# chunhualiao/Smith-Waterman

Hardware: AMD Instinct MI355X
Metric: GCUPS (DP cell updates/s) on NxN random DNA pair (higher is better)
Workload: dtype int32; 1 GPU; 16384x16384 random DNA pair (reference generator, seed 1+rank), linear gap 3/-3/-2, int32 H + int32 P written to HBM, arg-max tracked; per_gpu=one pair per GPU, max_pos=268369846, max_score=11583, grid=256, column_tiles=1, strips=131, placement_held_gib=0, preheat_fills=620

## Files before the change

### smith-waterman_amd/csrc/sw_api.hip

```cpp
#include <hip/hip_runtime.h>
#include <algorithm>
#include <chrono>
#include <cstdio>
#include <cstdlib>
#include <cstring>
#include <iterator>
#include <map>
#include <mutex>
#include <string>
#include <thread>
#include <vector>
#include "sw_kernels.h"
#include "sw_plan.h"

namespace swh { void set_err(const char* fmt, ...); }
extern "C" int sw_place_pair_ratio(void* d_X, size_t xbytes, void* d_Y, size_t ybytes, float* ratio, float* ms_together);
using swh::set_err;

#define HIP_TRY(expr)                                                                 \
    do {                                                                              \
        hipError_t e_ = (expr);                                                       \
        if (e_ != hipSuccess) {                                                       \
            set_err("%s failed: %s (%s:%d)", #expr, hipGetErrorString(e_), __FILE__, __LINE__); \
            return SW_EDEVICE;                                                        \
// ... 7 lines not shown
    hipEvent_t ev = nullptr;
    int concurrent_ok = 0;
};
static DevState g_dev[64];

struct sw_ctx {
    int device = 0;
    int num_cus = 256;
    unsigned epoch = 0;
    unsigned long long* d_edge = nullptr;
    size_t edge_cap = 0;
    unsigned long long* d_key = nullptr;
    unsigned long long* d_keys = nullptr; size_t keys_cap = 0;
    unsigned char* d_cb = nullptr;
    size_t cb_cap = 0;
    unsigned int* d_edge4 = nullptr;
    size_t edge4_cap = 0;
    unsigned epoch8 = 0;
    unsigned char* d_alpha = nullptr;
    unsigned int* d_part = nullptr;
    unsigned int* d_sync = nullptr;
    unsigned char* d_priv = nullptr; size_t priv_cap = 0;
    int64_t opt_place_hold_gib = 0;
    int64_t opt_place_budget_ms = 1500;
    int place_spacer_gib = 0;
    int64_t last_place_held_gib = 0;
    float last_place_ratio = 0.f;
    bool key_dirty = false;
    bool last_fused = false;
    swp::PlanOptions opt;
    swp::FillPlan last_plan;
    int64_t last_grid = 0;
    int s2_per_cu = 0;
    int64_t opt_xcd_order = 0;
    int64_t opt_pace_ps = 0;
    int64_t opt_dbg_ptr = 0;
    int64_t opt_band_wait_ms = 20000;
    unsigned char* d_bcodes = nullptr; size_t bcodes_cap = 0;
    int* d_bnd = nullptr; size_t bnd_cap = 0;
    int64_t opt_batch_lds = 0;
    int64_t last_batch_kernel = 0;
    signed char* d_sprof = nullptr; size_t sprof_cap = 0;
    int* d_sbnd = nullptr; size_t sbnd_cap = 0;
    swk::SearchItem* d_sitems = nullptr; swk::SearchItem* h_sitems = nullptr; size_t sitems_cap = 0;
    hipEvent_t sitems_ev = nullptr;
    unsigned int* d_sctr = nullptr;
    int64_t last_search_grid = 0;
    int64_t last_search_kernel = 0;
    int search_per_cu[swp::kSearchKernels] = {};
    bool search_per_cu_known = false;
    bool xcd_round_robin = false;
    std::map<void*, void*> out_base;
    std::map<void*, float> pair_ratio;
};

template <typename K> struct Indexed { int index; K k; };
template <typename K, size_t N> constexpr bool at_their_indices(const Indexed<K> (&t)[N]) {
    for (size_t i = 0; i < N; ++i)
        if (t[i].index != (int)i) return false;
    return true;
}

extern "C" {

int sw_create(int device, sw_ctx** out) {
    if (!out) { set_err("sw_create: out is NULL"); return SW_EINVAL; }
// ... 82 lines not shown
    if (!strcmp(name, "engine")) {
        if (v != 0 && v != 1) { set_err("engine must be 0 (systolic) or 1 (strip_scan)"); return SW_EINVAL; }
        c->opt.engine = v;
        return SW_OK;
    }
    set_err("sw_set_option: unknown option '%s'", name);
    return SW_EINVAL;
}

int64_t sw_get_option(sw_ctx* c, const char* name) {
    if (!c || !name) return -1;
    if (!strcmp(name, "waves_per_block")) return c->opt.waves_per_block;
    if (!strcmp(name, "max_blocks")) return c->opt.max_blocks;
    if (!strcmp(name, "engine")) return c->opt.engine;
    if (!strcmp(name, "strips_per_group")) return c->opt.strips_per_group;
    if (!strcmp(name, "consumers")) return c->opt.consumers;
    if (!strcmp(name, "store_policy")) return c->opt.store_policy;
    if (!strcmp(name, "xcd_order")) return c->opt_xcd_order;
    if (!strcmp(name, "importers")) return c->opt.importers;
    if (!strcmp(name, "pace_ps")) return c->opt_pace_ps;
    if (!strcmp(name, "band_wait_ms")) return c->opt_band_wait_ms;
    if (!strcmp(name, "num_cus")) return c->num_cus;
    if (!strcmp(name, "debug_edge4_ptr")) return (int64_t)(uintptr_t)c->d_edge4;
    if (!strcmp(name, "debug_edge4_cap")) return (int64_t)c->edge4_cap;
    if (!strcmp(name, "last_grid")) return c->last_grid;
    const swp::TilePlan& last_tile = c->last_plan.tile[c->last_plan.ntile - 1];
    if (!strcmp(name, "last_strips")) return c->last_plan.S;
    if (!strcmp(name, "last_strips2")) return last_tile.strips;
    if (!strcmp(name, "last_perm")) return c->last_plan.perm ? 1 : 0;
    if (!strcmp(name, "last_scouts")) return last_tile.nscout;
    if (!strcmp(name, "last_xcd_mode")) return last_tile.xcd_mode;
    if (!strcmp(name, "last_tiles")) return c->last_plan.ntile;
    if (!strcmp(name, "last_split_from")) return last_tile.split_blk ? last_tile.split_from : 0;
    if (!strcmp(name, "xcd_round_robin")) return c->xcd_round_robin ? 1 : 0;
    if (!strcmp(name, "last_batch_kernel")) return c->last_batch_kernel;
    if (!strcmp(name, "last_search_grid")) return c->last_search_grid;
    if (!strcmp(name, "last_search_kernel")) return c->last_search_kernel;
    if (!strcmp(name, "placement_budget_ms")) return c->opt_place_budget_ms;
    if (!strcmp(name, "placement_hold_gib")) return c->opt_place_hold_gib;
    if (!strcmp(name, "probe_foreign_pairs")) return c->opt.probe_foreign_pairs;
    if (!strcmp(name, "last_placement_held_gib")) return c->last_place_held_gib;
    if (!strcmp(name, "last_placement_ratio_x1000")) return (int64_t)(c->last_place_ratio * 1000.f);
    return -1;
}

static int check_dims(int64_t cols, int64_t rows, const sw_scores* sc, int64_t gc = -1, int64_t gr = -1) {
    if (gc < cols) gc = cols;
    if (gr < rows) gr = rows;
    if (cols < 0 || rows < 0 || cols > swk::SW_MAX_DIM || rows > swk::SW_MAX_DIM || gc > swk::SW_MAX_DIM || gr > swk::SW_MAX_DIM) {
        set_err("dimensions out of range: cols=%lld rows=%lld (max %lld)", (long long)cols, (long long)rows,
                (long long)swk::SW_MAX_DIM);
        return SW_EINVAL;
    }
    if (sc->gap > 0) { set_err("gap score must be <= 0 (got %d)", sc->gap); return SW_EINVAL; }
    if (sc->match < 0) { set_err("match score must be >= 0 (got %d)", sc->match); return SW_EINVAL; }
    if (sc->mismatch > sc->match) { set_err("mismatch score must not exceed the match score"); return SW_EINVAL; }
    const int64_t lo = std::min(gc, gr);
    const int64_t gmax = (int64_t)sc->match * lo + (int64_t)(-sc->gap) * (rows + cols + 2);
    const int64_t step = std::max<int64_t>(std::llabs((int64_t)sc->mismatch), (int64_t)sc->match) + 2 * (int64_t)(-sc->gap);
    if (gmax + step >= (1ll << 31) || step >= (1ll << 24) || (int64_t)sc->match * lo >= (1ll << 24)) {
        set_err("scores too large for this problem size (32-bit cell / 24-bit arg-max key)");
        return SW_EINVAL;
    }
    return SW_OK;
}

// ... 168 lines not shown
    unsigned short* d_cb16 = (unsigned short*)(c->d_cb + cb16);
    unsigned char* d_cbc = c->d_cb + cb16 + ((2 * c->cb_cap + 15) / 16) * 16;
    if (plan.perm) {
        p.edge4 = c->d_edge4; p.e4stride = plan.e4stride; p.edge4_pstride = S * plan.e4stride;
        p.gbias = next_gbias(c, stream);
    }
    p.bcode = d_cbc;
    p.atab = c->d_alpha + 64;
    p.phi_base = plan.fast ? (int)S - 1 : -1;
    p.bfront = (int)plan.bfront;
    p.bpad16 = d_cb16;
    p.bpad8 = c->d_cb;
    p.bpad_pstride = plan.per;
    if (plan.two_cols) {
        if (c->key_dirty) { HIP_TRY(hipMemsetAsync(c->d_key, 0, 16, stream)); c->key_dirty = false; }
        for (int64_t tile = 0; tile < plan.ntile; ++tile) {
            const swp::TilePlan& t = plan.tile[tile];
            swk::FillParams p2 = p;
            p2.nstrips = (int)t.strips; p2.cols = t.cols; p2.h_bytes = j.h_elem_bytes; p2.s2w = plan.W2; p2.store_nt = t.store_nt;
            p2.alpha_a = ua; p2.alpha_cols = cols;
            p2.idx_off = t.c0; p2.final_launch = tile + 1 == plan.ntile ? 1 : 0;
            if (plan.ntile > 1) {
                p2.H = (char*)j.d_H + t.c0 * 4; p2.P = (int32_t*)((char*)j.d_P + t.c0 * 4);
                p2.tile_left = tile ? (const int32_t*)j.d_H + t.c0 : nullptr;
                if (tile) p2.gbias = next_gbias(c, stream);
            }
            p2.nscout = t.nscout; p2.scout_double = t.scout_double; p2.xcd_mode = t.xcd_mode;
            p2.split_blk = t.split_blk; p2.split_from = t.split_from; p2.split_extra = t.split_extra;
            p2.filler_end_steps = t.filler_end_steps; p2.filler_full_steps = t.filler_full_steps;
            p2.filler_hop_ps = t.filler_hop_ps; p2.filler_tau_ps = t.filler_tau_ps; p2.filler_bw_gbs = t.filler_bw_gbs;
            p2.sync = c->d_sync; p2.priv = c->d_priv; p2.priv_stride = plan.priv_stride;
            p2.bpad16_w = d_cb16; p2.bpad8_w = c->d_cb; p2.bcode_w = d_cbc; p2.atab_w = c->d_alpha + 64;
            p2.result = j.d_result; p2.skip_row0 = (j.d_top || j.d_top_gran) ? 1 : 0;
            hipLaunchKernelGGL(kSystolic2[t.consumers - 4][plan.W2 == 110], dim3(t.grid), dim3(768), 0, stream, ua + t.c0, ub, p2);
        }
        p.skip_if_perm = 1;
        p.sync = c->d_sync; p.atab_w = c->d_alpha + 64; p.result = j.d_result; p.final_launch = 1;
        c->last_fused = true;
    } else {
        const int64_t total = (cols + rows) * j.npairs;
        const unsigned nscan = (unsigned)std::max<int64_t>(1, std::min<int64_t>((total + 1023) / 1024, 2048));
        hipLaunchKernelGGL(swk::sw_prep_scan, dim3(nscan), dim3(256), 0, stream, ua, cols, j.a_pstride, ub, rows, j.b_pstride, j.npairs, c->d_part);
        const unsigned npad = (unsigned)((plan.per + 255) / 256);
        hipLaunchKernelGGL(swk::sw_prep_code, dim3(npad, (unsigned)j.npairs), dim3(256), 0, stream, ub, rows, plan.bfront, j.b_pstride, c->d_cb, d_cb16,
                           d_cbc, (const unsigned int*)c->d_part, (int)nscan, c->d_alpha + 64, plan.per, (int)npad, (void*)nullptr, j.h_elem_bytes,
                           (void*)nullptr, j.p_elem_bytes, cols + 1, rows + 1, 0, j.zero_key ? j.d_keys : nullptr);
        c->key_dirty = true;
    }
    const SystolicKernel kern = j.h_elem_bytes == 4 ? one_col->h32 : one_col->h64;
    int per_cu = 0;
    HIP_TRY(hipOccupancyMaxActiveBlocksPerMultiprocessor(&per_cu, kern, plan.threads, 0));
    if (per_cu < 1) { set_err("the fill kernel does not fit a CU on this device"); return SW_EDEVICE; }
    c->last_grid = std::min<int64_t>(plan.grid, (int64_t)per_cu * c->num_cus);
    hipLaunchKernelGGL(kern, dim3((unsigned)c->last_grid), dim3(plan.threads), 0, stream, ua, ub, (const unsigned char*)c->d_cb, p);
    HIP_TRY(hipGetLastError());
    return SW_OK;
}

static const sw_scores kDefaultScores = {3, -3, -2};

static int fill_one(sw_ctx* c, const sw_scores* scores, FillJob j, int64_t gcols, int64_t grows, sw_result* d_result, void* stream_,
                    const char* who) {
    const sw_scores* sc = scores ? scores : &kDefaultScores;
    const int64_t cols = j.cols, rows = j.rows;
    if (!c || !d_result || (j.h_elem_bytes != 4 && j.h_elem_bytes != 8) || (j.p_elem_bytes != 4 && j.p_elem_bytes != 1) ||
        j.stride < cols + 1) {
        set_err("%s: bad argument", who);
        return SW_EINVAL;
    }
    if (int rc = check_dims(cols, rows, sc, gcols, grows)) return rc;
    if ((cols > 0 && !j.d_a) || (rows > 0 && !j.d_b)) { set_err("%s: NULL sequence", who); return SW_EINVAL; }
    hipStream_t stream = (hipStream_t)stream_;
    HIP_TRY(hipSetDevice(c->device));
    DevOrder order(c, stream, j.concurrent);
    if (order.rc) return order.rc;
    j.d_keys = c->d_key;
    j.d_result = d_result;
    j.zero_key = c->opt.engine == 0 && cols > 0 && rows > 0;
    if (!j.zero_key) { HIP_TRY(hipMemsetAsync(c->d_key, 0, 16, stream)); c->key_dirty = true; }
    c->last_fused = false;
    if (cols == 0 || rows == 0) {
        if (j.stride != cols + 1 || j.d_left || j.d_right || j.d_top_gran || j.d_bot_gran) { set_err("%s: empty tiles / bands are not supported", who); return SW_EINVAL; }
        const int64_t M = cols + 1;
        if (j.d_H) HIP_TRY(hipMemsetAsync(j.d_H, 0, (size_t)(M * (rows + 1)) * j.h_elem_bytes, stream));
// ... 692 lines not shown
```

### smith-waterman_amd/csrc/sw_debug.h

```cpp
#pragma once

namespace swk {

enum DebugFlag : int {
    DBG_NO_STORES = 1 << 0,
    DBG_PRODUCER_ONLY = 1 << 1,
    DBG_GENERIC_PRODUCER = 1 << 2,
    DBG_SKIP_STRIP1 = 1 << 3,
    DBG_NO_PERM = 1 << 4,
    DBG_NO_POLL_BACKOFF = 1 << 5,
    DBG_WAVE_PLACEMENT = 1 << 6,
    DBG_BLOCK_STAMPS = 1 << 7,
    DBG_NO_CONSUMER_LOOP = 1 << 8,
    DBG_EDGE_DUMP = 1 << 9,
    DBG_EPOCH8_WRAP_EARLY = 1 << 10,
    DBG_POISON_HALO = 1 << 11,
    DBG_ONE_IMPORTER = 1 << 12,
    DBG_PROGRESS_FORM = 1 << 13,
    DBG_NO_TWO_COLUMNS = 1 << 14,
    DBG_FORCE_TWO_COLUMNS = 1 << 15,
    DBG_BATCH_SINGLE_PAIR = 1 << 16,
    DBG_NO_SCOUTS = 1 << 17,
    DBG_BATCH_NO_WAVE16 = 1 << 18,
    DBG_NO_TILES = 1 << 19,
    DBG_NO_SPLIT = 1 << 20,
    DBG_BATCH_NO_PACKED_P = 1 << 21,
    DBG_S2_SCOUTS_NO_EXPORT = 1 << 21,
    DBG_S2_SYNTH_HALO = 1 << 22,
    DBG_NO_XCD_DEALING = 1 << 23,
    DBG_S2_IMPORTERS = 3 << 24,
    DBG_NO_PACING = 1 << 27,
};
constexpr int DBG_S2_IMPORTERS_SHIFT = 24;
constexpr int DBG_BATCH_MASK = DBG_NO_STORES | DBG_PRODUCER_ONLY | DBG_GENERIC_PRODUCER;

}
```

### smith-waterman_amd/csrc/sw_kernels.h

```cpp
#pragma once
#include <hip/hip_runtime.h>
#include <stdint.h>
#include "../../include/swhip.h"
#include "sw_plan.h"

namespace swk {

constexpr unsigned long long SW_KEY_IDX_MASK = (1ull << 40) - 1;
constexpr int64_t SW_MAX_DIM = (1 << 20) - 1;

struct FillParams {
    int64_t cols, rows, M;
    void* H;
    int32_t* P;
    const int32_t* top;
    const int32_t* left;
    int32_t* right;
    int npairs;
    int store_hp;
    int64_t a_pstride, b_pstride, bpad_pstride, hp_pstride, edge_pstride;
    int32_t mm, xm, ngap;
    unsigned long long* edge;
    unsigned int tag_base;
    unsigned long long* result_key;
// ... 12 lines not shown
    const unsigned long long* top_gran;
    unsigned long long* bot_gran;
    unsigned int* bot_done;
    unsigned int top_tag, bot_tag;
    unsigned int top_wait_ticks;
    const unsigned char* bcode;
    const unsigned char* atab;
    unsigned int* edge4;
    int64_t e4stride, edge4_pstride;
    unsigned int gbias;
    int skip_if_perm;
    int h_bytes;
    int scout_double;
    int nscout;
    int filler_hop_ps, filler_tau_ps, filler_bw_gbs;
    int xcd_mode;
    unsigned int* sync;
    unsigned char* priv;
    int64_t priv_stride;
    unsigned short* bpad16_w;
    unsigned char* bpad8_w; unsigned char* bcode_w; unsigned char* atab_w;
    sw_result* result;
    int skip_row0;
    const int32_t* tile_left;
    int64_t idx_off;
    int final_launch;
    const unsigned char* alpha_a;
    int64_t alpha_cols;
    int split_blk, split_from;
    int split_extra;
    int filler_end_steps;
    int filler_full_steps;
    int s2w;
};
constexpr int SW_XTAB_OFF = 448;
constexpr int SW_PERM_PAD = -100;

struct BatchParams {
    const unsigned char* a; int64_t a_pstride, cols;
    const unsigned char* bcode; int64_t bcode_pstride; int bfront;
    int64_t rows, npairs;
    const unsigned char* atab;
    int32_t* H; void* P;
    int64_t hp_pstride;
    int match, mismatch, ngap;
    int* bnd; int64_t bnd_pstride;
    sw_result* results;
    int debug;
};
__global__ void sw_batch_codes(const unsigned char* b, int64_t rows, int64_t b_pstride, unsigned char* bcode, int64_t per, int front,
                               const unsigned int* part, int npart, unsigned char* atab, int64_t npairs);
template <int C, int PB>
__global__ void sw_batch_wave(BatchParams p);
template <bool LE4, bool K12, bool PB1>
__global__ void sw_batch_wave16(BatchParams p);

struct SearchParams {
    const unsigned char* db;
    const SearchItem* items; int64_t nitems;
    const signed char* prof; int64_t qpad;
    int64_t qlen;
    int match, mismatch, ngap;
    int* bnd; int64_t bnd_per;
    unsigned int* counter;
    sw_result* results;
};
// ... 30 lines not shown
```

### smith-waterman_amd/csrc/sw_plan.cpp

```cpp
#include "sw_plan.h"
#include <algorithm>
#include <vector>

namespace swp {

constexpr double kOneStripPerCu = 4.5;
constexpr double kChainBoundCells = 3.5e8;
constexpr double kStreamCells = 6.0e8;
constexpr double kChainSecPerStrip = 3.1e-6, kHbmBytesPerSec = 3.2e12;
constexpr int64_t kScoutStrips = 170;
constexpr double kOneClassCells = 2.0e8;
constexpr float kOneClassRatio = 1.7f;
constexpr int64_t kTileStrips = 160;
constexpr double kTileHopSec = 2.4e-6, kTileRowSec = 26e-9, kTileBytesPerSec = 3.0e12;
constexpr double kClassicHopSec = 7.6e-6, kClassicRowSec = 35e-9, kClassicBytesPerSec = 3.3e12;
constexpr double kTileGain = 0.98;
constexpr int64_t kXcdChainStrips = 384;
constexpr double kScoutLeadSec = 21.5e-9;
constexpr int64_t kSplitRows = 4096;

constexpr int64_t kC4Cols = 256, kC8Cols = 512;
constexpr int64_t kBndSlackRows = 160;
constexpr int64_t kWaveSlackRows = 132;
constexpr double kWaveMatrixBytes = 2147483648.0;
// ... 136 lines not shown
            const Deal d = deal_per_xcd(S2, false);
            if (d.fits) { t.xcd_mode = 1; t.nscout = d.scouts; t.scout_double = d.doubles; t.grid = 256; }
        }
        if (t.xcd_mode == 1 && (rows >= kSplitRows || o.split_blk > 0) && !j.has_top && !j.has_top_gran && !j.has_bot_gran && o.filler_hop_ps > 0 &&
            !(o.debug_flags & (DBG_NO_PACING | DBG_NO_SPLIT))) {
            const Deal d = deal_per_xcd(S2, true);
            const double hop = (double)o.filler_hop_ps * 1e-12, tf = (double)o.filler_tau_ps * 1e-12, ts = kScoutLeadSec;
            const int64_t nblk = (rows + 15) / 16;
            const int64_t sblk = (int64_t)((double)nblk * tf / (2.0 * tf - std::min(ts, tf)));
            const bool forced = o.split_blk > 0;
            if (d.fits && forced && o.split_blk < nblk) {
                t.split_blk = (int)o.split_blk; t.split_from = (int)std::max<int64_t>(1, o.split_from); t.split_extra = 1;
                t.filler_end_steps = (int)((o.split_blk * 16 + 126) / 64 * 64 + 64); t.filler_full_steps = (int)((nblk * 16 + 126) / 64 * 64 + 64);
                t.nscout = d.scouts; t.scout_double = d.doubles;
            } else if (d.fits && sblk >= 16 && sblk < nblk && rows >= kSplitRows) {
                const int64_t full_steps = (nblk * 16 + 126) / 64 * 64 + 64, end_steps = (sblk * 16 + 126) / 64 * 64 + 64;
                const double lead = ((double)full_steps - (double)end_steps) * tf / hop;
                const int64_t from = std::max<int64_t>(1, (int64_t)((double)(S2 - 1) - lead) + 1);
                if (from < S2) {
                    t.split_blk = (int)sblk; t.split_from = (int)from; t.split_extra = 1;
                    t.filler_end_steps = (int)end_steps; t.filler_full_steps = (int)full_steps;
                    t.nscout = d.scouts; t.scout_double = d.doubles;
                }
            }
        }
        const bool xcd_chain_pays = S2 >= kXcdChainStrips && W2 != 110;
        if (!scouts && dev.xcd_round_robin && t.grid >= 64 && !(o.debug_flags & DBG_NO_XCD_DEALING) &&
            (o.xcd_chain == 1 || (o.xcd_chain == 0 && xcd_chain_pays)))
            t.xcd_mode = 2;
        t.filler_hop_ps = (scouts && !(o.debug_flags & DBG_NO_PACING)) ? (int)o.filler_hop_ps : 0;
        t.filler_tau_ps = (int)o.filler_tau_ps;
        t.filler_bw_gbs = (int)o.filler_bw_gbs;
        t.consumers = o.consumers == 0 ? ((scouts || W2 == 110) ? 7 : (chain_bound ? 5 : 6)) : (int)std::min<int64_t>(7, o.consumers);
    }
    return f;
}

namespace {
int lane_columns(int64_t cols) { return cols <= kC4Cols ? 4 : cols <= kC8Cols ? 8 : 16; }
int64_t boundary_ints(int64_t nstrips, int64_t rows) { return nstrips > 1 ? ((rows + kBndSlackRows + 3) / 4) * 4 : 0; }
}

BatchPlan plan_batch(const BatchJob& j, const PlanOptions& o) {
    using namespace swk;
    BatchPlan b;
    const int64_t cols = j.cols, rows = j.rows;
    b.wave = !(o.debug_flags & DBG_BATCH_SINGLE_PAIR) && j.match <= kWaveScore && j.match >= -kWaveScore && j.mismatch <= kWaveScore &&
             j.mismatch >= -kWaveScore && (double)(rows + kWaveSlackRows) * (double)(cols + 1) * 4.0 < kWaveMatrixBytes;
    b.single_chunk = std::min(j.npairs, kSingleChunk);
    b.C = lane_columns(cols);
    b.nstrips = (cols + 64 * b.C - 1) / (64 * b.C);
    b.front = kCodesFront;
    b.per = ((rows + kCodesFront + kCodesTail + 15) / 16) * 16;
    b.bnd_per = boundary_ints(b.nstrips, rows);
    b.chunk = std::max<int64_t>(1, std::min<int64_t>(j.npairs, std::min<int64_t>(kBatchWorkspaceBytes / b.per,
                                                                                  b.bnd_per ? kBatchWorkspaceBytes / (b.bnd_per * 4) : j.npairs)));
    b.grid = (b.chunk + 3) / 4;
    b.scan_blocks = (int)std::max<int64_t>(1, std::min<int64_t>(((cols + rows) * j.npairs + kScanLetters - 1) / kScanLetters, kScanBlocks));
    b.codes_blocks = (int)std::min<int64_t>((b.per + 255) / 256, kCodesBlocks);
    b.bcodes_need = (size_t)(b.chunk * b.per);
    b.bnd_need = (size_t)(b.chunk * b.bnd_per);
    const int64_t smax = (int64_t)j.match * std::min(cols, rows);
    b.fits16 = j.npairs >= 2 && b.C == 16 && smax < kWave16Score && -j.gap < kWave16Score && rows < kWave16Rows && !(o.debug_flags & DBG_BATCH_NO_WAVE16);
    b.k12 = smax < kKeyedScore;
    b.packed16 = b.fits16 && !j.has_H && (!j.has_P || (j.p_elem_bytes == 1 && !(o.debug_flags & DBG_BATCH_NO_PACKED_P)));
    return b;
// ... 40 lines not shown
```

### smith-waterman_amd/csrc/sw_plan.h

```cpp
#pragma once
#include <cstddef>
#include <cstdint>
#include "sw_debug.h"

namespace swk {

constexpr int SW_SEARCH_ROWS = 257;
struct SearchItem { int64_t start, idx, len; };

}

namespace swp {

struct PlanJob {
    int64_t cols = 0, rows = 0, npairs = 1;
    bool full_stride = true;
    int h_elem_bytes = 4, p_elem_bytes = 4;
    bool has_H = true, has_P = true;
    bool has_top = false;
    bool has_left = false, has_right = false;
    bool has_top_gran = false, has_bot_gran = false;
    bool has_result = true;
    int64_t total_rows = 0;
    int reserve_cus = 0;
    bool h_aligned = true, p_aligned = true;
    int match = 3, mismatch = -3, gap = -2;
    float pair_ratio = 0.f;
};

constexpr int kSearchKernels = 6;
constexpr int search_kernel_index(int C, bool wide) { return 2 * (C / 8) + wide; }

struct DeviceFacts {
    int num_cus = 256;
    bool xcd_round_robin = false;
    int s2_per_cu = 0;
    int search_per_cu[kSearchKernels] = {};
};

struct PlanOptions {
    int64_t engine = 0, strips_per_group = 0, consumers = 0, importers = 0, max_blocks = 0, waves_per_block = 4, store_policy = 0;
    int64_t s2w = 0, xcd_chain = 0, split_blk = 0, split_from = 0;
    int64_t filler_hop_ps = 2400000, filler_tau_ps = 25000, filler_bw_gbs = 4200;
    int64_t probe_foreign_pairs = 0, debug_flags = 0;
};

struct TilePlan {
    int64_t c0 = 0, cols = 0, strips = 0;
    int grid = 0, nscout = 0, scout_double = 0, xcd_mode = 0;
    int split_blk = 0, split_from = 0, split_extra = 0, filler_end_steps = 0, filler_full_steps = 0;
    int filler_hop_ps = 0, filler_tau_ps = 0, filler_bw_gbs = 0;
    int store_nt = 0;
    int consumers = 0;
};

constexpr int kMaxTiles = 64;

struct FillPlan {
    int engine = 0;
    int64_t S = 0;
    int store_nt = 0;
    int NS = 0, NC = 0, importers = 0, threads = 0;
    int grid = 0;
    bool fast = false;
    int64_t bfront = 0, per = 0;
    bool perm = false;
    int64_t e4stride = 0;
    bool two_cols = false;
    int W2 = 126;
    int64_t ntile = 1, tstrips = 0;
    TilePlan tile[kMaxTiles];
    int64_t priv_stride = 0;
    size_t edge_need = 0, cb_need = 0, edge4_need = 0, priv_need = 0;
    size_t h_bytes = 0, p_bytes = 0;
    bool probe_pair_class = false;
};

FillPlan plan_fill(const PlanJob& job, const DeviceFacts& dev, const PlanOptions& opt);

struct BatchJob {
    int64_t cols = 0, rows = 0, npairs = 1;
    bool has_H = true, has_P = true;
    int p_elem_bytes = 4;
    int match = 3, mismatch = -3, gap = -2;
};

struct BatchPlan {
    bool wave = false;
    int C = 0;
    int64_t nstrips = 0;
    int front = 0;
    int64_t per = 0;
    int64_t bnd_per = 0;
    int64_t chunk = 0;
    int64_t grid = 0;
    int scan_blocks = 0, codes_blocks = 0;
    bool fits16 = false, k12 = false, packed16 = false;
    size_t bcodes_need = 0, bnd_need = 0;
    int64_t single_chunk = 0;
};

BatchPlan plan_batch(const BatchJob& job, const PlanOptions& opt);

constexpr int kBatchWave16 = 9, kBatchKernels = 17;
constexpr int batch_wave_index(int C, int pb) { return 3 * (C / 8) + (pb == 4 ? 2 : pb); }
constexpr int batch_wave16_index(bool le4, bool k12, bool pb1) { return kBatchWave16 + 4 * le4 + 2 * k12 + pb1; }
int batch_kernel(const BatchPlan& plan, unsigned nletters, int64_t n, int p_bytes);

struct SearchJob {
    int64_t qlen = 0, maxlen = 0;
    int64_t ntargets = 0;
// ... 20 lines not shown
```

### smith-waterman_amd/csrc/sw_systolic2.inc

```

constexpr int S2_W = 126;
template <bool OV> __device__ __forceinline__ constexpr int s2_stride() { return OV ? 110 : S2_W; }
template <bool OV> __device__ __forceinline__ constexpr int s2_xlane() { return s2_stride<OV>() >> 1; }

struct S2Side {
    __attribute__((aligned(16))) u32 halo[SY_RH];
    __attribute__((aligned(16))) u32 lowv[128];
    int topv[128];
    int prod_u, halo_ready, never, pad;
};
struct Sys2Lds {
    __attribute__((aligned(16))) unsigned char ringA[64 * SY_LSTR];
    __attribute__((aligned(16))) unsigned char ringB[64 * SY_LSTR];
    __attribute__((aligned(16))) int cons_blk[8];
    S2Side side;
};

#define P2_STEP(GA, GB, GA1, GB1, TAP, TAN, TBP, TBN, HIN, SA, SB, BYTE)                                                   \
    "v_add_u32 v121, v121, %[ngap]\n\t"                                                                                   \
    "v_max3_i32 v120, " TBP ", " GB1 ", v121\n\t"                                                                         \
    "v_max3_i32 v122, " TAP ", " GB1 ", v121\n\t"                                                                         \
    "v_add_u32_sdwa " TBN ", " GB1 ", sext(" SA ") dst_sel:DWORD dst_unused:UNUSED_PAD src0_sel:DWORD src1_sel:" BYTE "\n\t" \
    "v_max_i32_dpp " GA ", v120, " GA1 " wave_shr:1 row_mask:0xf bank_mask:0xf\n\t"                                       \
    "v_max3_i32 " GB ", v122, " GA ", " HIN "\n\t"                                                                        \
// ... 413 lines not shown
    const int jA = s * s2_stride<OV>() + 2 * lane - 1, jB = jA + 1;
    const int topA = lane >= 1 ? sd.topv[2 * lane - 1] : 0, topB = sd.topv[2 * lane];
    const int jn = jA + 2;
    const u32 ca = (lane < 63 && jn >= 1 && jn <= p.cols) ? (u32)ltab[seq_a[jn - 1]] : 8u;
    const u32 cb = (lane >= 1 && jB <= p.cols) ? (u32)ltab[seq_a[jB - 1]] : 8u;
    u32 palo = 0, pahi = 0, pblo = 0, pbhi = 0;
#pragma unroll
    for (int c = 0; c < 4; ++c) {
        palo |= ((u32)(unsigned char)(signed char)((u32)c == ca ? mm : xm)) << (8 * c);
        pblo |= ((u32)(unsigned char)(signed char)((u32)c == cb ? mm : xm)) << (8 * c);
    }
#pragma unroll
    for (int c = 4; c < 7; ++c) {
        pahi |= ((u32)(unsigned char)(signed char)((u32)c == ca ? mm : xm)) << (8 * (c - 4));
        pbhi |= ((u32)(unsigned char)(signed char)((u32)c == cb ? mm : xm)) << (8 * (c - 4));
    }
    pahi |= ((u32)(unsigned char)(signed char)SW_PERM_PAD) << 24;
    pbhi |= ((u32)(unsigned char)(signed char)SW_PERM_PAD) << 24;
    if (lane == 0) {
        const u32 pad4 = 0x01010101u * (u32)(unsigned char)(signed char)SW_PERM_PAD;
        pblo = pad4; pbhi = pad4;
    }
    const u32 ga1 = lane == 0 ? (u32)gb : (u32)(gb + topA + ngap * (int)jA), gb1 = (u32)(gb + topB + ngap * (int)jB);
    const u32 z0 = (u32)(gb + ngap * (1 - phi - lane + (int)jA));
    const unsigned char* cbase = bcode + (p.bfront - phi - 64);
    const u32 expoff = (exports && s + 1 < S && lane == s2_xlane<OV>()) ? 0u : SY_OOB;
    const uint64_t eb = (uint64_t)(uintptr_t)(p.edge4 + (int64_t)s * p.e4stride);
    const sw_i32x4p erc = {(int)(u32)eb, (int)(u32)(eb >> 32), 0x7FFFFF00, 0x00020000};
    int polls[2];
    u64* const dbg = p.dbg ? p.dbg + ((!SCOUT && p.nscout > 0 && !stamps_as_scout) ? 6 * p.nstrips + 32 : 0) : nullptr;
    if (dbg && lane == 0) {
        dbg[2 * s] = __builtin_amdgcn_s_memrealtime();
        if (s == 0 && dbg == p.dbg) p.dbg[6 * p.nstrips + 16] = __builtin_amdgcn_s_memtime();
    }
    int st;
    if constexpr (SCOUT) {
        if constexpr (LOCAL) {
            st = producer_scout2_local(palo, pahi, pblo, pbhi, (u32)ngap, 63u - (u32)lane, z0, ga1, gb1, ga1 + (u32)SW_PERM_PAD, gb1 + (u32)SW_PERM_PAD, expoff, cbase,
                                       (u32)(size_t)&sd.halo[0], (u32)(size_t)&sd.lowv[0], (u32)(size_t)&sd.prod_u, UT, erc, polls);
        } else
            st = producer_scout2(palo, pahi, pblo, pbhi, (u32)ngap, 63u - (u32)lane, z0, ga1, gb1, ga1 + (u32)SW_PERM_PAD, gb1 + (u32)SW_PERM_PAD, expoff, cbase,
                                 (u32)(size_t)&sd.halo[0], (u32)(size_t)&sd.lowv[0], (u32)(size_t)&sd.prod_u, UT, erc, polls);
    } else {
        const u32 wA = (u32)(size_t)&full->ringA[0] + (u32)lane * (u32)SY_LSTR, wB = (u32)(size_t)&full->ringB[0] + (u32)lane * (u32)SY_LSTR;
        const int kc = 30 - SY_R - phi, kr = -SY_R - phi - 32;
        if (ua >= 0)
            st = producer_scoutfill2(palo, pahi, pblo, pbhi, (u32)ngap, wA, wB, 63u - (u32)lane, z0, ga1, gb1, ga1 + (u32)SW_PERM_PAD, gb1 + (u32)SW_PERM_PAD,
                                     local_rt ? SY_OOB : expoff, local_rt ? expoff : SY_OOB, cbase, (u32)(size_t)&sd.halo[0], (u32)(size_t)&sd.lowv[0],
                                     (u32)(size_t)&full->cons_blk[0], (u32)(size_t)&sd.never, (u32)(size_t)&sd.prod_u, ua, UT, kc, kr, erc, polls);
        else
        st = producer_perm2(palo, pahi, pblo, pbhi, (u32)ngap, wA, wB, 63u - (u32)lane, z0, ga1, gb1, ga1 + (u32)SW_PERM_PAD, gb1 + (u32)SW_PERM_PAD,
                            local_rt ? SY_OOB : expoff, local_rt ? expoff : SY_OOB, cbase, (u32)(size_t)&sd.halo[0], (u32)(size_t)&sd.lowv[0],
                            (u32)(size_t)&full->cons_blk[0], (u32)(size_t)&sd.never, (u32)(size_t)&sd.prod_u, UT, kc, kr, erc, polls);
    }
    if (dbg && lane == 0) {
        dbg[2 * s + 1] = __builtin_amdgcn_s_memrealtime();
        if (s == 0 && dbg == p.dbg) p.dbg[6 * p.nstrips + 17] = __builtin_amdgcn_s_memtime();
        if (dbg == p.dbg) {
            dbg[4 * p.nstrips + 16 + 2 * s] = (u64)polls[0];
            dbg[4 * p.nstrips + 17 + 2 * s] = (u64)polls[1];
        }
    }
    return st;
}

struct XcdLayout { int f0, nf, s0, ns, ndx, w; };
// ... 12 lines not shown
    for (int x = 0; x < 8; ++x) {
        const XcdLayout l = xcd_layout(S, x, extra);
        if (t >= l.s0 && t < l.s0 + l.ns && t <= S - 2 + extra) return t - l.s0 >= 2 * l.ndx;
    }
    return false;
}
__device__ __forceinline__ bool xcd_local_readers(const FillParams& p, int S, int s, unsigned my_xcc, int far_block, Spin& spin, bool& local) {
    const u32* xtab = (const u32*)(p.atab + SW_XTAB_OFF);
    int blocks[3] = {-1, -1, far_block};
    for (int x = 0; x < 8; ++x) {
        const XcdLayout l = xcd_layout(S, x, p.split_extra);
        const int t = s + 1;
        if (t >= l.f0 && t < l.f0 + l.nf) blocks[0] = 8 * (l.w + t - l.f0) + x;
        if (t <= S - 2 + p.split_extra && t >= l.s0 && t < l.s0 + l.ns) blocks[1] = 8 * ((t - l.s0 < 2 * l.ndx) ? (t - l.s0) / 2 : t - l.s0 - l.ndx) + x;
    }
    local = true;
    for (int i = 0; i < 3; ++i) {
        if (blocks[i] < 0) continue;
        u32 v;
        while ((v = __hip_atomic_load((gu32*)(xtab + blocks[i]), __ATOMIC_RELAXED, __HIP_MEMORY_SCOPE_AGENT)) == 0u)
            if (spin.fail(p.abort_flag)) return false;
        local = local && v == my_xcc + 1u;
    }
    return true;
}

struct S2Prep {
    __attribute__((aligned(16))) unsigned char tab[256];
    unsigned int pres[8];
    int nletters, ok;
};
constexpr int S2_SYNC_BAR = 0, S2_SYNC_OUT = 1, S2_SYNC_MAP = 8;

__device__ __forceinline__ int s2_prologue(S2Prep& pp, const FillParams& p, const unsigned char* __restrict__ seq_a, const unsigned char* __restrict__ seq_b) {
    const int tid = (int)threadIdx.x, nth = (int)blockDim.x, G = (int)gridDim.x, wg = (int)blockIdx.x;
    gu32* const sync = (gu32*)p.sync;
    if (tid < 8) pp.pres[tid] = 0u;
    __syncthreads();
    {
        const int64_t acols = p.alpha_cols, total = acols + p.rows, chunk = (total + G - 1) / G;
        const int64_t lo = (int64_t)wg * chunk, hi = min(total, lo + chunk);
        for (int64_t i = lo + tid; i < hi; i += nth) {
            const unsigned char ch = i < acols ? p.alpha_a[i] : seq_b[i - acols];
            atomicOr(&pp.pres[ch >> 5], 1u << (ch & 31));
        }
    }
    __syncthreads();
    if (tid < 64) {
        if (tid < 8 && pp.pres[tid]) (void)__hip_atomic_fetch_or(sync + S2_SYNC_MAP + tid, pp.pres[tid], __ATOMIC_RELAXED, __HIP_MEMORY_SCOPE_AGENT);
        __builtin_amdgcn_fence(__ATOMIC_RELEASE, "agent");
        if (tid == 0) (void)__hip_atomic_fetch_add(sync + S2_SYNC_BAR, 1u, __ATOMIC_RELAXED, __HIP_MEMORY_SCOPE_AGENT);
        Spin spin; spin.code = 17;
        bool ok = true;
        while ((u32)__builtin_amdgcn_readfirstlane((int)__hip_atomic_load(sync + S2_SYNC_BAR, __ATOMIC_RELAXED, __HIP_MEMORY_SCOPE_AGENT)) < (u32)G)
            if (spin.fail(p.abort_flag)) { ok = false; break; }
        if (tid < 8) pp.pres[tid] = __hip_atomic_load(sync + S2_SYNC_MAP + tid, __ATOMIC_RELAXED, __HIP_MEMORY_SCOPE_AGENT);
        if (tid == 0) pp.ok = ok ? 1 : 0;
    }
    __syncthreads();
    if (!pp.ok) return -1;
    if (tid < 256) {
        int rank = 0, nl = 0;
#pragma unroll
        for (int w = 0; w < 8; ++w) {
            const unsigned int m = pp.pres[w];
            nl += __popc(m);
            if (w < (tid >> 5)) rank += __popc(m);
            else if (w == (tid >> 5)) rank += __popc(m & ((1u << (tid & 31)) - 1u));
        }
        const bool here = (pp.pres[tid >> 5] >> (tid & 31)) & 1u;
        pp.tab[tid] = (here && nl <= 7) ? (unsigned char)rank : (unsigned char)7;
        if (tid == 0) pp.nletters = nl;
    }
    __syncthreads();
    const int nl = pp.nletters;
    const int64_t per = p.bpad_pstride, front = p.bfront, rows = p.rows;
    if (wg == 0) {
        if (tid < 256) p.atab_w[tid] = pp.tab[tid];
        if (tid == 0) *(unsigned int*)(p.atab_w + 256) = (unsigned int)nl;
        if (nl > 7)
            for (int64_t i = tid; i < per; i += nth) {
                const bool in = (i >= front && i - front < rows);
                const unsigned char ch = in ? seq_b[i - front] : (unsigned char)0;
                p.bpad8_w[i] = ch;
                p.bpad16_w[i] = in ? (unsigned short)ch : (unsigned short)0x100;
                p.bcode_w[i] = (unsigned char)7;
            }
    }
    if (nl <= 7) {
        unsigned char* const mine = p.priv + (int64_t)wg * p.priv_stride;
        for (int64_t i = 4 * (int64_t)tid; i < per; i += 4 * (int64_t)nth) {
            const int64_t k = i - front;
            u32 raw = 0u, code = 0x07070707u;
            if (k >= 0 && k + 4 <= rows) {
                raw = *(const u32*)(seq_b + k);
                code = (u32)pp.tab[raw & 255u] | ((u32)pp.tab[(raw >> 8) & 255u] << 8) | ((u32)pp.tab[(raw >> 16) & 255u] << 16) | ((u32)pp.tab[raw >> 24] << 24);
            } else if (k + 4 > 0 && k < rows) {
#pragma unroll
                for (int q = 0; q < 4; ++q)
                    if (k + q >= 0 && k + q < rows) {
                        const u32 ch = seq_b[k + q];
                        raw |= ch << (8 * q);
                        code = (code & ~(0xffu << (8 * q))) | ((u32)pp.tab[ch] << (8 * q));
                    }
            }
            *(u32*)(mine + i) = raw;
            *(u32*)(mine + per + i) = code;
        }
        const int64_t M = p.M, nrow0 = p.cols + 1, nedge = nrow0 + rows, chunk = (nedge + G - 1) / G;
        const int64_t lo = (int64_t)wg * chunk, hi = min(nedge, lo + chunk);
        void* const H = p.H; void* const P = (void*)p.P;
        const bool own_col0 = p.tile_left == nullptr;
        for (int64_t e = lo + tid; e < hi; e += nth) {
            if (e < nrow0) {
                if (!p.skip_row0 && (e > 0 || own_col0)) {
                    if (H) { if (p.h_bytes == 8) ((int64_t*)H)[e] = 0; else ((int32_t*)H)[e] = 0; }
                    if (P) { if (p.p_bytes == 1) ((signed char*)P)[e] = 0; else ((int32_t*)P)[e] = 0; }
                }
            } else if (own_col0) {
                const int64_t r = e - nrow0 + 1;
                if (H) { if (p.h_bytes == 8) ((int64_t*)H)[r * M] = 0; else ((int32_t*)H)[r * M] = 0; }
                if (P) { if (p.p_bytes == 1) ((signed char*)P)[r * M] = 0; else ((int32_t*)P)[r * M] = 0; }
            }
        }
    }
    __builtin_amdgcn_fence(__ATOMIC_RELEASE, "workgroup");
    __syncthreads();
    __builtin_amdgcn_fence(__ATOMIC_ACQUIRE, "workgroup");
    return nl;
}

__device__ __forceinline__ void s2_epilogue(const FillParams& p, bool worked) {
    asm volatile("s_waitcnt vmcnt(0)" ::: "memory");
    __syncthreads();
    if (threadIdx.x != 0) return;
    gu32* const sync = (gu32*)p.sync;
    const u32 prev = __hip_atomic_fetch_add(sync + S2_SYNC_OUT, 1u, __ATOMIC_RELAXED, __HIP_MEMORY_SCOPE_AGENT);
    if (prev != gridDim.x - 1u) return;
    if (worked && p.final_launch) {
        const u64 k = __hip_atomic_load((gu64*)p.result_key, __ATOMIC_RELAXED, __HIP_MEMORY_SCOPE_AGENT);
        const u32 ab = __hip_atomic_load((gu32*)p.abort_flag, __ATOMIC_RELAXED, __HIP_MEMORY_SCOPE_AGENT);
        if (p.result) {
            p.result->max_score = (int64_t)(k >> 40);
            p.result->max_pos = k ? (int64_t)(SW_KEY_IDX_MASK - (k & SW_KEY_IDX_MASK)) : 0;
            p.result->path_len = ab ? -(int64_t)ab : 0;
        }
        __hip_atomic_store((gu64*)p.result_key, 0ull, __ATOMIC_RELAXED, __HIP_MEMORY_SCOPE_AGENT);
        __hip_atomic_store((gu32*)p.abort_flag, 0u, __ATOMIC_RELAXED, __HIP_MEMORY_SCOPE_AGENT);
    }
    if (worked) {
        gu32* const xtab = (gu32*)(p.atab_w + SW_XTAB_OFF);
        for (int i = 0; i < 256; ++i) __hip_atomic_store(xtab + i, 0u, __ATOMIC_RELAXED, __HIP_MEMORY_SCOPE_AGENT);
    }
    for (int w = 0; w < 8; ++w) __hip_atomic_store(sync + S2_SYNC_MAP + w, 0u, __ATOMIC_RELAXED, __HIP_MEMORY_SCOPE_AGENT);
    __hip_atomic_store(sync + S2_SYNC_BAR, 0u, __ATOMIC_RELAXED, __HIP_MEMORY_SCOPE_AGENT);
    __hip_atomic_store(sync + S2_SYNC_OUT, 0u, __ATOMIC_RELAXED, __HIP_MEMORY_SCOPE_AGENT);
}

template <int NC, bool OV>
__device__ __forceinline__ void s2_body(Sys2Lds& lds, const unsigned char* ltab, const unsigned char* my_bpad8, const unsigned char* my_bcode,
                                        const unsigned char* seq_a, const FillParams& p) {
    const int lane = threadIdx.x & 63;
    const int wave = __builtin_amdgcn_readfirstlane((int)(threadIdx.x >> 6));
    const int64_t M = p.M;
    const int rows = (int)p.rows;
    const int ngap = p.ngap, mm = p.mm, xm = p.xm;
    const int S = p.nstrips;
    const int gb = (int)p.gbias;
    const int nscout = p.nscout;

    int sc_cnt = 0, sc_s0 = 0, sc_far = -1, sc_far_block = -1, fill_s = S, fill_step = S;
    unsigned my_xcc = 0;
    if (p.xcd_mode == 1) {
        const int x = (int)blockIdx.x & 7, k = (int)blockIdx.x >> 3;
        const XcdLayout l = xcd_layout(S, x, p.split_extra);
        const int nf = l.nf, f0 = l.f0, s0 = l.s0, ns = l.ns, ndx = l.ndx, w = l.w;
        asm volatile("s_getreg_b32 %0, hwreg(HW_REG_XCC_ID)" : "=s"(my_xcc));
        my_xcc &= 15u;
        if (threadIdx.x == 0) __hip_atomic_store((gu32*)(p.atab + SW_XTAB_OFF) + blockIdx.x, my_xcc + 1u, __ATOMIC_RELAXED, __HIP_MEMORY_SCOPE_AGENT);
        if (k < w) {
            sc_cnt = k < ndx ? 2 : 1;
            sc_s0 = s0 + (k < ndx ? 2 * k : k + ndx);
            sc_far = s0 + ns - 1;
            sc_far_block = 8 * ((ns - 1 < 2 * ndx) ? (ns - 1) / 2 : ns - 1 - ndx) + x;
        } else if (k - w < nf) {
            fill_s = f0 + k - w;
        } else {
            return;
        }
// ... 372 lines not shown
```

Before: 331.4 GCUPS.

## Replace grid-wide alphabet barrier with per-block full scan for small inputs

For inputs whose combined length fits a threshold, each workgroup now scans both sequences on its own with 16-byte vector loads to build the alphabet bitmap. This removes the grid-wide atomic barrier that used to merge per-block bitmaps. The prologue's padded code build moves from 4-byte to 16-byte chunks, the epilogue reset is spread across a wavefront, and occupancy queries are cached per kernel instantiation. The cost is redundant global reads of the sequences by every block; debug timestamps are also added.

```diff
diff --git a/smith-waterman_amd/csrc/sw_api.hip b/smith-waterman_amd/csrc/sw_api.hip
--- a/smith-waterman_amd/csrc/sw_api.hip
+++ b/smith-waterman_amd/csrc/sw_api.hip
@@ -63,6 +63,7 @@
     swp::FillPlan last_plan;
     int64_t last_grid = 0;
     int s2_per_cu = 0;
+    struct { int threads, per_cu; } sys_occ[8][2] = {};
     int64_t opt_xcd_order = 0;
     int64_t opt_pace_ps = 0;
     int64_t opt_dbg_ptr = 0;
@@ -211,6 +212,7 @@
     if (!strcmp(name, "last_xcd_mode")) return last_tile.xcd_mode;
     if (!strcmp(name, "last_tiles")) return c->last_plan.ntile;
     if (!strcmp(name, "last_split_from")) return last_tile.split_blk ? last_tile.split_from : 0;
+    if (!strcmp(name, "last_scan_all")) return last_tile.scan_all;
     if (!strcmp(name, "xcd_round_robin")) return c->xcd_round_robin ? 1 : 0;
     if (!strcmp(name, "last_batch_kernel")) return c->last_batch_kernel;
     if (!strcmp(name, "last_search_grid")) return c->last_search_grid;
@@ -445,6 +447,7 @@
             p2.sync = c->d_sync; p2.priv = c->d_priv; p2.priv_stride = plan.priv_stride;
             p2.bpad16_w = d_cb16; p2.bpad8_w = c->d_cb; p2.bcode_w = d_cbc; p2.atab_w = c->d_alpha + 64;
             p2.result = j.d_result; p2.skip_row0 = (j.d_top || j.d_top_gran) ? 1 : 0;
+            p2.scan_all = t.scan_all;
             hipLaunchKernelGGL(kSystolic2[t.consumers - 4][plan.W2 == 110], dim3(t.grid), dim3(768), 0, stream, ua + t.c0, ub, p2);
         }
         p.skip_if_perm = 1;
@@ -461,8 +464,13 @@
         c->key_dirty = true;
     }
     const SystolicKernel kern = j.h_elem_bytes == 4 ? one_col->h32 : one_col->h64;
-    int per_cu = 0;
-    HIP_TRY(hipOccupancyMaxActiveBlocksPerMultiprocessor(&per_cu, kern, plan.threads, 0));
+    static_assert(sizeof(kSystolic) / sizeof(kSystolic[0]) == 8, "sw_ctx::sys_occ has one row per instantiation");
+    auto& occ = c->sys_occ[one_col - std::begin(kSystolic)][j.h_elem_bytes == 4 ? 0 : 1];
+    if (occ.threads != plan.threads) {
+        HIP_TRY(hipOccupancyMaxActiveBlocksPerMultiprocessor(&occ.per_cu, kern, plan.threads, 0));
+        occ.threads = plan.threads;
+    }
+    const int per_cu = occ.per_cu;
     if (per_cu < 1) { set_err("the fill kernel does not fit a CU on this device"); return SW_EDEVICE; }
     c->last_grid = std::min<int64_t>(plan.grid, (int64_t)per_cu * c->num_cus);
     hipLaunchKernelGGL(kern, dim3((unsigned)c->last_grid), dim3(plan.threads), 0, stream, ua, ub, (const unsigned char*)c->d_cb, p);
diff --git a/smith-waterman_amd/csrc/sw_debug.h b/smith-waterman_amd/csrc/sw_debug.h
--- a/smith-waterman_amd/csrc/sw_debug.h
+++ b/smith-waterman_amd/csrc/sw_debug.h
@@ -30,6 +30,8 @@
     DBG_NO_XCD_DEALING = 1 << 23,
     DBG_S2_IMPORTERS = 3 << 24,
     DBG_NO_PACING = 1 << 27,
+    DBG_S2_BARRIER_SCAN = 1 << 28,
+    DBG_S2_SCAN_ALL = 1 << 29,
 };
 constexpr int DBG_S2_IMPORTERS_SHIFT = 24;
 constexpr int DBG_BATCH_MASK = DBG_NO_STORES | DBG_PRODUCER_ONLY | DBG_GENERIC_PRODUCER;
diff --git a/smith-waterman_amd/csrc/sw_kernels.h b/smith-waterman_amd/csrc/sw_kernels.h
--- a/smith-waterman_amd/csrc/sw_kernels.h
+++ b/smith-waterman_amd/csrc/sw_kernels.h
@@ -68,6 +68,7 @@
     int filler_end_steps;
     int filler_full_steps;
     int s2w;
+    int scan_all;
 };
 constexpr int SW_XTAB_OFF = 448;
 constexpr int SW_PERM_PAD = -100;
diff --git a/smith-waterman_amd/csrc/sw_plan.cpp b/smith-waterman_amd/csrc/sw_plan.cpp
--- a/smith-waterman_amd/csrc/sw_plan.cpp
+++ b/smith-waterman_amd/csrc/sw_plan.cpp
@@ -192,6 +192,9 @@
         t.filler_tau_ps = (int)o.filler_tau_ps;
         t.filler_bw_gbs = (int)o.filler_bw_gbs;
         t.consumers = o.consumers == 0 ? ((scouts || W2 == 110) ? 7 : (chain_bound ? 5 : 6)) : (int)std::min<int64_t>(7, o.consumers);
+        t.scan_all = (cols + rows <= kScanAllLetters) ? 1 : 0;
+        if (o.debug_flags & DBG_S2_BARRIER_SCAN) t.scan_all = 0;
+        if (o.debug_flags & DBG_S2_SCAN_ALL) t.scan_all = 1;
     }
     return f;
 }
diff --git a/smith-waterman_amd/csrc/sw_plan.h b/smith-waterman_amd/csrc/sw_plan.h
--- a/smith-waterman_amd/csrc/sw_plan.h
+++ b/smith-waterman_amd/csrc/sw_plan.h
@@ -52,6 +52,7 @@
     int filler_hop_ps = 0, filler_tau_ps = 0, filler_bw_gbs = 0;
     int store_nt = 0;
     int consumers = 0;
+    int scan_all = 0;
 };
 
 constexpr int kMaxTiles = 64;
@@ -77,6 +78,8 @@
 };
 
 FillPlan plan_fill(const PlanJob& job, const DeviceFacts& dev, const PlanOptions& opt);
+
+constexpr int64_t kScanAllLetters = 48 * 1024;
 
 struct BatchJob {
     int64_t cols = 0, rows = 0, npairs = 1;
diff --git a/smith-waterman_amd/csrc/sw_systolic2.inc b/smith-waterman_amd/csrc/sw_systolic2.inc
--- a/smith-waterman_amd/csrc/sw_systolic2.inc
+++ b/smith-waterman_amd/csrc/sw_systolic2.inc
@@ -469,6 +469,7 @@
     if (dbg && lane == 0) {
         dbg[2 * s] = __builtin_amdgcn_s_memrealtime();
         if (s == 0 && dbg == p.dbg) p.dbg[6 * p.nstrips + 16] = __builtin_amdgcn_s_memtime();
+        if (s == 0 && dbg == p.dbg) p.dbg[8 * p.nstrips + 32 + 3] = dbg[0];
     }
     int st;
     if constexpr (SCOUT) {
@@ -547,32 +548,80 @@
 };
 constexpr int S2_SYNC_BAR = 0, S2_SYNC_OUT = 1, S2_SYNC_MAP = 8;
 
+enum { S2_STAMP_ENTRY = 0, S2_STAMP_ALPHABET = 1, S2_STAMP_PROLOGUE = 2, S2_STAMP_FIRST_STEP = 3, S2_STAMP_STORES = 4, S2_STAMP_OUT = 5, S2_STAMP_LAST_ENTRY = 6 };
+__device__ __forceinline__ void s2_stamp(const FillParams& p, int k, bool is_max) {
+    u64* const slot = p.dbg + 8 * p.nstrips + 32 + k;
+    const u64 now = __builtin_amdgcn_s_memrealtime();
+    if (is_max) (void)__hip_atomic_fetch_max(slot, now, __ATOMIC_RELAXED, __HIP_MEMORY_SCOPE_AGENT);
+    else *slot = now;
+}
+
+__device__ __forceinline__ void s2_scan_all(S2Prep& pp, const unsigned char* __restrict__ seq, int64_t n, int tid, int nth) {
+    if (n <= 0) return;
+    const uintptr_t a0 = (uintptr_t)seq & ~(uintptr_t)15;
+    const int64_t skew = (int64_t)((uintptr_t)seq - a0), nchunk = (skew + n + 15) >> 4;
+    u32 cw = 8u, cm = 0u;
+    for (int64_t c0 = tid; c0 < nchunk; c0 += 4 * (int64_t)nth) {
+        uint4 v[4];
+#pragma unroll
+        for (int u = 0; u < 4; ++u) {
+            const int64_t c = c0 + (int64_t)u * nth;
+            v[u] = c < nchunk ? *(const uint4*)(a0 + 16 * (uintptr_t)c) : make_uint4(0u, 0u, 0u, 0u);
+        }
+#pragma unroll
+        for (int u = 0; u < 4; ++u) {
+            const int64_t c = c0 + (int64_t)u * nth;
+            if (c >= nchunk) break;
+            const u32 w[4] = {v[u].x, v[u].y, v[u].z, v[u].w};
+            const int64_t first = skew - 16 * c, end = skew + n - 16 * c;
+            const bool whole = first <= 0 && end >= 16;
+#pragma unroll
+            for (int q = 0; q < 16; ++q) {
+                if (!whole && (q < first || q >= end)) continue;
+                const u32 ch = (w[q >> 2] >> (8 * (q & 3))) & 255u;
+                const u32 bit = 1u << (ch & 31u);
+                if ((ch >> 5) != cw) { cw = ch >> 5; cm = __hip_atomic_load(&pp.pres[cw], __ATOMIC_RELAXED, __HIP_MEMORY_SCOPE_WORKGROUP); }
+                if (!(cm & bit)) { atomicOr(&pp.pres[cw], bit); cm |= bit; }
+            }
+        }
+    }
+}
+
 __device__ __forceinline__ int s2_prologue(S2Prep& pp, const FillParams& p, const unsigned char* __restrict__ seq_a, const unsigned char* __restrict__ seq_b) {
     const int tid = (int)threadIdx.x, nth = (int)blockDim.x, G = (int)gridDim.x, wg = (int)blockIdx.x;
     gu32* const sync = (gu32*)p.sync;
+    if (p.dbg && wg == 0 && tid == 0) s2_stamp(p, S2_STAMP_ENTRY, false);
+    if (p.dbg && tid == 0) s2_stamp(p, S2_STAMP_LAST_ENTRY, true);
     if (tid < 8) pp.pres[tid] = 0u;
+    if (tid == 0) pp.ok = 1;
     __syncthreads();
-    {
-        const int64_t acols = p.alpha_cols, total = acols + p.rows, chunk = (total + G - 1) / G;
-        const int64_t lo = (int64_t)wg * chunk, hi = min(total, lo + chunk);
-        for (int64_t i = lo + tid; i < hi; i += nth) {
-            const unsigned char ch = i < acols ? p.alpha_a[i] : seq_b[i - acols];
-            atomicOr(&pp.pres[ch >> 5], 1u << (ch & 31));
+    if (p.scan_all) {
+        s2_scan_all(pp, p.alpha_a, p.alpha_cols, tid, nth);
+        s2_scan_all(pp, seq_b, p.rows, tid, nth);
+    } else {
+        {
+            const int64_t acols = p.alpha_cols, total = acols + p.rows, chunk = (total + G - 1) / G;
+            const int64_t lo = (int64_t)wg * chunk, hi = min(total, lo + chunk);
+            for (int64_t i = lo + tid; i < hi; i += nth) {
+                const unsigned char ch = i < acols ? p.alpha_a[i] : seq_b[i - acols];
+                atomicOr(&pp.pres[ch >> 5], 1u << (ch & 31));
+            }
+        }
+        __syncthreads();
+        if (tid < 64) {
+            if (tid < 8 && pp.pres[tid]) (void)__hip_atomic_fetch_or(sync + S2_SYNC_MAP + tid, pp.pres[tid], __ATOMIC_RELAXED, __HIP_MEMORY_SCOPE_AGENT);
+            __builtin_amdgcn_fence(__ATOMIC_RELEASE, "agent");
+            if (tid == 0) (void)__hip_atomic_fetch_add(sync + S2_SYNC_BAR, 1u, __ATOMIC_RELAXED, __HIP_MEMORY_SCOPE_AGENT);
+            Spin spin; spin.code = 17;
+            bool ok = true;
+            while ((u32)__builtin_amdgcn_readfirstlane((int)__hip_atomic_load(sync + S2_SYNC_BAR, __ATOMIC_RELAXED, __HIP_MEMORY_SCOPE_AGENT)) < (u32)G)
+                if (spin.fail(p.abort_flag)) { ok = false; break; }
+            if (tid < 8) pp.pres[tid] = __hip_atomic_load(sync + S2_SYNC_MAP + tid, __ATOMIC_RELAXED, __HIP_MEMORY_SCOPE_AGENT);
+            if (tid == 0) pp.ok = ok ? 1 : 0;
         }
     }
     __syncthreads();
-    if (tid < 64) {
-        if (tid < 8 && pp.pres[tid]) (void)__hip_atomic_fetch_or(sync + S2_SYNC_MAP + tid, pp.pres[tid], __ATOMIC_RELAXED, __HIP_MEMORY_SCOPE_AGENT);
-        __builtin_amdgcn_fence(__ATOMIC_RELEASE, "agent");
-        if (tid == 0) (void)__hip_atomic_fetch_add(sync + S2_SYNC_BAR, 1u, __ATOMIC_RELAXED, __HIP_MEMORY_SCOPE_AGENT);
-        Spin spin; spin.code = 17;
-        bool ok = true;
-        while ((u32)__builtin_amdgcn_readfirstlane((int)__hip_atomic_load(sync + S2_SYNC_BAR, __ATOMIC_RELAXED, __HIP_MEMORY_SCOPE_AGENT)) < (u32)G)
-            if (spin.fail(p.abort_flag)) { ok = false; break; }
-        if (tid < 8) pp.pres[tid] = __hip_atomic_load(sync + S2_SYNC_MAP + tid, __ATOMIC_RELAXED, __HIP_MEMORY_SCOPE_AGENT);
-        if (tid == 0) pp.ok = ok ? 1 : 0;
-    }
-    __syncthreads();
+    if (p.dbg && tid == 0) s2_stamp(p, S2_STAMP_ALPHABET, true);
     if (!pp.ok) return -1;
     if (tid < 256) {
         int rank = 0, nl = 0;
@@ -604,23 +653,26 @@
     }
     if (nl <= 7) {
         unsigned char* const mine = p.priv + (int64_t)wg * p.priv_stride;
-        for (int64_t i = 4 * (int64_t)tid; i < per; i += 4 * (int64_t)nth) {
+        for (int64_t i = 16 * (int64_t)tid; i < per; i += 16 * (int64_t)nth) {
             const int64_t k = i - front;
-            u32 raw = 0u, code = 0x07070707u;
-            if (k >= 0 && k + 4 <= rows) {
-                raw = *(const u32*)(seq_b + k);
-                code = (u32)pp.tab[raw & 255u] | ((u32)pp.tab[(raw >> 8) & 255u] << 8) | ((u32)pp.tab[(raw >> 16) & 255u] << 16) | ((u32)pp.tab[raw >> 24] << 24);
-            } else if (k + 4 > 0 && k < rows) {
-#pragma unroll
-                for (int q = 0; q < 4; ++q)
+            u32 raw[4] = {0u, 0u, 0u, 0u}, code[4] = {0x07070707u, 0x07070707u, 0x07070707u, 0x07070707u};
+            if (k >= 0 && k + 16 <= rows) {
+                const uint4 v = *(const uint4*)(seq_b + k);
+                raw[0] = v.x; raw[1] = v.y; raw[2] = v.z; raw[3] = v.w;
+#pragma unroll
+                for (int d = 0; d < 4; ++d)
+                    code[d] = (u32)pp.tab[raw[d] & 255u] | ((u32)pp.tab[(raw[d] >> 8) & 255u] << 8) | ((u32)pp.tab[(raw[d] >> 16) & 255u] << 16) | ((u32)pp.tab[raw[d] >> 24] << 24);
+            } else if (k + 16 > 0 && k < rows) {
+#pragma unroll
+                for (int q = 0; q < 16; ++q)
                     if (k + q >= 0 && k + q < rows) {
                         const u32 ch = seq_b[k + q];
-                        raw |= ch << (8 * q);
-                        code = (code & ~(0xffu << (8 * q))) | ((u32)pp.tab[ch] << (8 * q));
-                    }
-            }
-            *(u32*)(mine + i) = raw;
-            *(u32*)(mine + per + i) = code;
+                        raw[q >> 2] |= ch << (8 * (q & 3));
+                        code[q >> 2] = (code[q >> 2] & ~(0xffu << (8 * (q & 3)))) | ((u32)pp.tab[ch] << (8 * (q & 3)));
+                    }
+            }
+            *(uint4*)(mine + i) = make_uint4(raw[0], raw[1], raw[2], raw[3]);
+            *(uint4*)(mine + per + i) = make_uint4(code[0], code[1], code[2], code[3]);
         }
         const int64_t M = p.M, nrow0 = p.cols + 1, nedge = nrow0 + rows, chunk = (nedge + G - 1) / G;
         const int64_t lo = (int64_t)wg * chunk, hi = min(nedge, lo + chunk);
@@ -642,17 +694,21 @@
     __builtin_amdgcn_fence(__ATOMIC_RELEASE, "workgroup");
     __syncthreads();
     __builtin_amdgcn_fence(__ATOMIC_ACQUIRE, "workgroup");
+    if (p.dbg && tid == 0) s2_stamp(p, S2_STAMP_PROLOGUE, true);
     return nl;
 }
 
 __device__ __forceinline__ void s2_epilogue(const FillParams& p, bool worked) {
     asm volatile("s_waitcnt vmcnt(0)" ::: "memory");
+    if (p.dbg && (threadIdx.x & 63u) == 0) s2_stamp(p, S2_STAMP_STORES, true);
     __syncthreads();
-    if (threadIdx.x != 0) return;
+    if (threadIdx.x >= 64) return;
+    const int lane = (int)threadIdx.x;
     gu32* const sync = (gu32*)p.sync;
-    const u32 prev = __hip_atomic_fetch_add(sync + S2_SYNC_OUT, 1u, __ATOMIC_RELAXED, __HIP_MEMORY_SCOPE_AGENT);
-    if (prev != gridDim.x - 1u) return;
-    if (worked && p.final_launch) {
+    u32 prev = 0u;
+    if (lane == 0) prev = __hip_atomic_fetch_add(sync + S2_SYNC_OUT, 1u, __ATOMIC_RELAXED, __HIP_MEMORY_SCOPE_AGENT);
+    if ((u32)__builtin_amdgcn_readfirstlane((int)prev) != gridDim.x - 1u) return;
+    if (lane == 0 && worked && p.final_launch) {
         const u64 k = __hip_atomic_load((gu64*)p.result_key, __ATOMIC_RELAXED, __HIP_MEMORY_SCOPE_AGENT);
         const u32 ab = __hip_atomic_load((gu32*)p.abort_flag, __ATOMIC_RELAXED, __HIP_MEMORY_SCOPE_AGENT);
         if (p.result) {
@@ -665,11 +721,15 @@
     }
     if (worked) {
         gu32* const xtab = (gu32*)(p.atab_w + SW_XTAB_OFF);
-        for (int i = 0; i < 256; ++i) __hip_atomic_store(xtab + i, 0u, __ATOMIC_RELAXED, __HIP_MEMORY_SCOPE_AGENT);
-    }
-    for (int w = 0; w < 8; ++w) __hip_atomic_store(sync + S2_SYNC_MAP + w, 0u, __ATOMIC_RELAXED, __HIP_MEMORY_SCOPE_AGENT);
-    __hip_atomic_store(sync + S2_SYNC_BAR, 0u, __ATOMIC_RELAXED, __HIP_MEMORY_SCOPE_AGENT);
-    __hip_atomic_store(sync + S2_SYNC_OUT, 0u, __ATOMIC_RELAXED, __HIP_MEMORY_SCOPE_AGENT);
+#pragma unroll
+        for (int i = 0; i < 256; i += 64) __hip_atomic_store(xtab + i + lane, 0u, __ATOMIC_RELAXED, __HIP_MEMORY_SCOPE_AGENT);
+    }
+    if (lane < 8) __hip_atomic_store(sync + S2_SYNC_MAP + lane, 0u, __ATOMIC_RELAXED, __HIP_MEMORY_SCOPE_AGENT);
+    if (lane == 0) {
+        __hip_atomic_store(sync + S2_SYNC_BAR, 0u, __ATOMIC_RELAXED, __HIP_MEMORY_SCOPE_AGENT);
+        __hip_atomic_store(sync + S2_SYNC_OUT, 0u, __ATOMIC_RELAXED, __HIP_MEMORY_SCOPE_AGENT);
+        if (p.dbg) s2_stamp(p, S2_STAMP_OUT, false);
+    }
 }
 
 template <int NC, bool OV>
```

Result: faster. 337.7 GCUPS (median of 6 runs) (+1.9%).
